# openzklib/openzl

Hardware: AMD Instinct MI355X
Metric: MSM points/sec (BLS12-381 G1) (higher is better)
Workload: dtype u32; 1 GPU; bls12_381_g1_msm_2^24_per_gpu; points_per_gpu=16777216, curve=BLS12-381 G1, scalars=uniform < r (255 bit), window_bits=20, windows=13, precomputed_table=none (the fixed-key table mode is reported separately as msm_fixed_key), parallelism=single

## Files before the change

openzl_amd/backend.py:

```python
from __future__ import annotations

import collections
import ctypes as C
import os
from typing import Optional, Tuple

import numpy as np

HERE = os.path.dirname(os.path.abspath(__file__))
LIB_PATH = os.path.join(HERE, "libzl_backend.so")

ZL_BLS12_381, ZL_BN254 = 1, 2
ZL_G1, ZL_G2 = 1, 2
ZL_MONT, ZL_COSET, ZL_INVERSE, ZL_CHECK, ZL_MONT_IN, ZL_MONT_OUT = 1, 2, 4, 8, 16, 32
ZL_PARTIAL_WORDS = 64
CURVES = {"bls12_381": ZL_BLS12_381, "bn254": ZL_BN254}
FQ_LIMBS = {ZL_BLS12_381: 6, ZL_BN254: 4}

u64p = C.POINTER(C.c_uint64)
u8p = C.POINTER(C.c_uint8)
i32p = C.POINTER(C.c_int32)

ABI_SYMBOLS = [
    "zl_ctx_create", "zl_ctx_destroy", "zl_ctx_fork", "zl_ctx_set_stream", "zl_ctx_sync", "zl_ctx_set_msm_window", "zl_ctx_last_hip_error",
# ... 744 lines not shown
            self.L.zl_mctx_destroy(self._m)
            self._m = C.c_void_p()

    def __del__(self):
        try:
            self.close()
        except Exception:
            pass


TEST_ABI_SYMBOLS = ["zl_test_poseidon_permute_dev", "zl_test_fp28_op", "zl_test_fp28_bn_op", "zl_test_pairing_product", "zl_test_point_op", "zl_test_circuit_tweak", "zl_test_fq_mul_rate", "zl_test_fr28_op", "zl_test_fr29_op",
                    "zl_test_poseidon_permute_dev28r", "zl_test_fq_mul_clock", "zl_test_acc_clock", "zl_test_acc_clock_read", "zl_test_clock_probe_launch", "zl_test_clock_probe_read",
                    "zl_test_miller_dev", "zl_test_final_exp", "zl_test_verify_batch_host", "zl_test_ntt_plan", "zl_test_ntt_fit_beside", "zl_test_fp2pair_op", "zl_test_point_form_op",
                    "zl_test_endo_split", "zl_test_endo_split_inf", "zl_test_decode_points_host", "zl_test_fq2_sqrt",
                    "zl_test_final_exp_dev", "zl_test_fq12_inverse", "zl_test_fq12_zeta", "zl_test_pairing_product_scaled",
                    "zl_test_msm_plan", "zl_test_msm_batch_form"]


def _p32(a: np.ndarray):
    assert a.dtype == np.uint32 and a.flags["C_CONTIGUOUS"]
    return a.ctypes.data_as(C.POINTER(C.c_uint32))


def groth16_keys_parse(curve: int, data: bytes, check: bool = False) -> int:
    buf = (C.c_uint8 * max(1, len(data))).from_buffer_copy(data if data else b"\0")
    return int(load_library().zl_groth16_keys_parse(curve, buf, len(data), ZL_CHECK if check else 0))


def hook_ntt_plan(log_n: int) -> list[int]:
    P = C.c_uint(0)
    sizes = (C.c_uint * 4)()
    rc = load_library().zl_test_ntt_plan(log_n, C.byref(P), sizes)
    if rc != 0:
        raise BackendError(rc, "zl_test_ntt_plan")
    assert all(sizes[k] == 0 for k in range(P.value, 4))
    return [int(sizes[k]) for k in range(P.value)]


def hook_ntt_fit_beside(be: "Backend", on: bool) -> bool:
    old = be.L.zl_test_ntt_fit_beside(be._ctx, int(on))
    if old < 0:
        raise BackendError(old, "zl_test_ntt_fit_beside")
    return bool(old)


def hook_endo_split(be: "Backend", curve: int, group: int, scalars: np.ndarray, inf: Optional[np.ndarray] = None):
    s = np.ascontiguousarray(scalars, dtype=np.uint64)
    n = s.shape[0]
    assert s.shape == (n, 4)
    out = np.zeros(4 * n * 8 + 1, dtype=np.uint32)
    k, bits = C.c_int(0), C.c_int(0)
    tail = [C.c_size_t, C.POINTER(C.c_uint32), C.POINTER(C.c_int), C.POINTER(C.c_int)]
    be.L.zl_test_endo_split.argtypes = [C.c_void_p, C.c_int, C.c_int, u64p] + tail
    be.L.zl_test_endo_split_inf.argtypes = [C.c_void_p, C.c_int, C.c_int, u64p, u8p] + tail
    if inf is None:
        rc = be.L.zl_test_endo_split(be._ctx, curve, group, _p64(s), n, _p32(out), C.byref(k), C.byref(bits))
    else:
        f = np.ascontiguousarray(inf, dtype=np.uint8)
# ... 741 lines not shown
```

openzl_amd/csrc/zl_capi.hip:

```cpp
#include <stdio.h>
#include <stdlib.h>
#include <string.h>
#include <algorithm>
#include <new>
#include <thread>
#include <vector>
#include "zl_ctx.h"
#include "zl_pool.h"
#include "zl_msm_multi_plan.h"

zl_pool& zl_pool_get() {
    static zl_pool pool(std::min(7u, std::max(1u, std::thread::hardware_concurrency()) - 1u));
    return pool;
}

int zl_ctx_aux_init(zl_ctx* ctx) {
    for (zl_ctx** ax : {&ctx->aux, &ctx->aux2}) {
        if (*ax) continue;
        zl_ctx* a = new (std::nothrow) zl_ctx();
        if (!a) return ZL_ENOMEM;
        a->device = ctx->device;
        a->cu_count = ctx->cu_count;
        int prio_lo = 0, prio_hi = 0;
        (void)hipDeviceGetStreamPriorityRange(&prio_lo, &prio_hi);
// ... 60 lines not shown
    ctx->stream = ctx->own_stream;
    const int rc_s = zl_ctx_streams_init(ctx);
    if (rc_s) { zl_ctx_destroy(ctx); return rc_s; }
    *out = ctx;
    return ZL_OK;
}

int zl_ctx_fork(zl_ctx* parent, zl_ctx** out) {
    if (!parent || !out) return ZL_EINVAL;
    *out = nullptr;
    if (parent->parent) return ZL_EINVAL;
    zl_ctx* c = nullptr;
    const int rc = zl_ctx_create(&c, parent->device);
    if (rc) return rc;
    c->msm_c = parent->msm_c;
    {
        std::unique_lock<std::shared_mutex> lk(parent->maps_mu);
        c->parent = parent;
        c->next_handle = ((uint64_t)(++parent->fork_seq) << 48) | 1;
        parent->fork_list.push_back(c);
        parent->forks.fetch_add(1);
    }
    *out = c;
    return ZL_OK;
}

int zl_ctx_drop_lanes(zl_ctx* ctx) {
    if (!ctx) return ZL_EINVAL;
    if (ctx->pipeline_busy.load()) return ZL_EINVAL;
    zl_ctx* l = ctx->stream_lane_ctx;
// ... 326 lines not shown
```

openzl_amd/csrc/zl_ctx.h:

```cpp
#pragma once
#include <hip/hip_runtime.h>
#include <stdint.h>
#include <stdlib.h>
#include <algorithm>
#include <atomic>
#include <functional>
#include <initializer_list>
#include <map>
#include <memory>
#include <mutex>
#include <shared_mutex>
#include <vector>
#include "../../include/zl_backend_ext.h"
#include "zl_curve.h"
#include "zl_pool.h"

#define ZL_HIP(ctx, call)                                   \
    do {                                                    \
        hipError_t e_ = (call);                             \
        if (e_ != hipSuccess) {                             \
            (ctx)->last_hip = (int)e_;                      \
            return e_ == hipErrorOutOfMemory ? ZL_ENOMEM : ZL_EHIP; \
        }                                                   \
    } while (0)
// ... 148 lines not shown
    size_t nnz[3] = {0, 0, 0};
    int curve = 0;
};
struct zl_ctx {
    zl_ctx* parent = nullptr;
    std::atomic<int> forks{0};
    mutable std::shared_mutex maps_mu;
    std::vector<zl_ctx*> fork_list;
    int fork_seq = 0;
    int device = 0;
    int cu_count = 0;
    hipStream_t stream = nullptr;
    hipStream_t own_stream = nullptr;
    int last_hip = 0;
    int msm_c = 0;
    int timing_on = 0;
    zl_timing timing{};
    hipEvent_t ev[4] = {nullptr, nullptr, nullptr, nullptr};
    std::map<uint64_t, zl_bases> bases;
    std::map<uint64_t, zl_r1cs_dev> r1cs;
    uint64_t next_handle = 1;
    zl_scratch scratch[ZL_SLOT_COUNT];
    std::map<uint64_t, zl_twiddles> twiddles;
    size_t ntt_last_bytes = 0;
    std::vector<hipEvent_t> ev_pool[2];
    std::atomic<int> pipeline_busy{0};
    uint64_t ntt_clock = 0;
    hipStream_t stream_sort = nullptr;
    hipStream_t stream_lane[4] = {nullptr, nullptr, nullptr, nullptr};
    hipStream_t stream_tail[3] = {nullptr, nullptr, nullptr};
// ... 125 lines not shown
```

openzl_amd/csrc/zl_msm_job.h:

```cpp
#pragma once
#include <chrono>
#include <stdlib.h>
#include <string.h>
#include <stdio.h>
#include <algorithm>
#include <vector>
#include "zl_ctx.h"
#include "zl_pool.h"
#include "zl_msm_sort.h"
#include "zl_msm_endo.h"
#include "zl_msm_accumulate.h"
#include "zl_msm_reduce.h"

#ifndef ZL_GLS_HOLE_LO_LOG
#define ZL_GLS_HOLE_LO_LOG 11
#define ZL_GLS_HOLE_HI_LOG 17
#define ZL_GLS_END_LOG 19
#endif
static_assert(ZL_GLS_HOLE_LO_LOG >= 0 && ZL_GLS_HOLE_LO_LOG <= ZL_GLS_HOLE_HI_LOG && ZL_GLS_HOLE_HI_LOG <= ZL_GLS_END_LOG && ZL_GLS_END_LOG <= 32, "split below 2^END outside [2^LO, 2^HI)");

static int zl_pick_window(size_t n, int sc_bits, bool wide16 = false ) {
    const double per_bucket = (double)zl_tune("ZL_TUNE_BUCKET_COST_X10", sc_bits > 200 ? 45 : 52) / 10.0;
    double best = 1e300;
    int best_c = 2;
// ... 9 lines not shown

static int zl_pick_window_half(size_t n_points) {
    if (n_points < 2) return 0;
    int lg = 63 - __builtin_clzll((unsigned long long)n_points);
    if ((double)n_points >= 1.4142 * (double)((size_t)1 << lg)) lg++;
    static const signed char best[9] = {9, 0, 11, 12, 0, 0, 0, 16, 0};
    return lg >= 11 && lg <= 19 ? best[lg - 11] : 0;
}
static int zl_pick_window_quarter(size_t n_points) {
    if (n_points < 2) return 0;
    int lg = 63 - __builtin_clzll((unsigned long long)n_points);
    if ((double)n_points >= 1.4142 * (double)((size_t)1 << lg)) lg++;
    static const signed char best[9] = {9, 0, 11, 12, 13, 13, 13, 13, 14};
    return lg >= 10 && lg <= 18 ? best[lg - 10] : 0;
}

static int zl_pick_window_precomp(size_t n, int sc_bits) {
    if (n < (size_t)700000) return 16;
    if (n < ((size_t)1 << 21)) return 20;
    double best = 1e300;
    int best_c = 16;
    for (int c = 20; c <= 23; c++) {
        int W = (sc_bits + 1 + c - 1) / c;
        double cost = (double)n * W + 6.0 * (double)(1u << (c - 1));
        if (cost < best) { best = cost; best_c = c; }
    }
    return best_c;
}

struct MsmSortLayout {
// ... 1 lines not shown
    uint32_t nslices = 0, per_slice = 0;
    size_t hi8 = 0, part_lo = 0, part_idx = 0, pcounts = 0, idx2 = 0, counts2 = 0;
    uint32_t P = 0, pscan_blocks = 0, fsl = 0, P2 = 0, p2scan_blocks = 0;
    size_t slice_counts = 0;
    size_t vs = 0;
};
template <class G>
struct MsmJob {
    using F = typename G::F;
    using X = XYZZ<F>;
    bool pre = false;
    int c = 0, W = 0;
    int spread_t = -1;
    bool wide = false;
    bool glv = false;
    bool phi_cached = false;
    bool phi_owner = false;
    int sc_bits = 0, endo_k = 1;
    zl_slot phi_slot = ZL_SLOT_PHI_ONE_KEY;
    MsmSortLayout lay;
    unsigned char *d_sort_a = nullptr, *d_sort_b = nullptr;
    size_t n_real = 0;
    uint32_t* d_vs = nullptr;
    const Affine<F>* d_phi = nullptr;
    uint32_t H = 0, SETS = 0, NB = 0, ZL_CHUNK = 0, nchunks = 0, scan_blocks = 0, max_big = 0, max_giant = 0, Gn = 0, big_span = ZL_BIG_SPAN;
    uint32_t red_g0 = 0, red_lg0 = 0, red_blocks = 0, red_levels = 0;
    uint32_t roots_per_set = 0;
    uint64_t maxE = 0;
    size_t n = 0, first = 0;
    const zl_bases* bsp = nullptr;
// ... 16 lines not shown
    int plan(zl_ctx* ctx, const zl_bases& bs, size_t first_, const void* d_scalars, size_t n_, zl_slot phi_slot_) {
        static const bool no_glv = getenv("ZL_NO_GLV") != nullptr;
        bool try_glv = false;
        static const size_t glv_max = (size_t)1 << zl_tune("ZL_TUNE_GLV_MAX_LOG", 19);
        if constexpr (G::GLV) try_glv = bs.precomp_c == 0 && !no_glv && n_ >= 1 && n_ <= glv_max && (uint64_t)n_ * G::ENDO_K < (1ull << 31);
        if constexpr (G::GLV && G::ENDO_K == 2) {
            if constexpr (G::GLVP::LATTICE) {
                if (n_ >= ((size_t)1 << 13) && n_ < ((size_t)1 << 17)) try_glv = false;
            }
        }
        if constexpr (G::GLV && G::ENDO_K == 4) {
            if constexpr (G::GLVP::LATTICE) {
                if (((uint64_t)n_ >= (1ull << ZL_GLS_HOLE_LO_LOG) && (uint64_t)n_ < (1ull << ZL_GLS_HOLE_HI_LOG)) || (uint64_t)n_ >= (1ull << ZL_GLS_END_LOG)) try_glv = false;
            }
        }
        int rc = plan_as(ctx, bs, first_, d_scalars, n_, try_glv);
        if (!rc && glv && c <= 3) rc = plan_as(ctx, bs, first_, d_scalars, n_, false);
        if (!rc && glv && !wide && c > 16) rc = plan_as(ctx, bs, first_, d_scalars, n_, false);
        phi_slot = phi_slot_;
        phi_owner = glv;
        return rc;
    }
    int plan_as(zl_ctx* ctx, const zl_bases& bs, size_t first_, const void* d_scalars, size_t n_, bool glv_) {
        glv = glv_;
        n_real = n_;
        endo_k = glv ? (int)G::ENDO_K : 1;
        n = (size_t)endo_k * n_;
        sc_bits = !glv ? (int)G::SC_BITS : MsmJobPartBits<G>::value;
        first = first_;
        bsp = &bs;
        pre = bs.precomp_c > 0;
        c = pre ? bs.precomp_c : (ctx->msm_c > 0 ? ctx->msm_c : zl_pick_window(n, sc_bits, glv && G::ENDO_K != 2));
        if (!pre && ctx->msm_c <= 0 && glv) {
            int h = 0;
            if constexpr (G::ENDO_K == 2) {
                if (!G::GLVP::LATTICE) h = zl_pick_window_half(n_);
            } else {
                h = zl_pick_window_quarter(n_);
            }
            if (h) c = h;
        }
        if (c < 2) c = 2;
        if (c > 24) c = 24;
        W = (sc_bits + 1 + c - 1) / c;
        H = 1u << (c - 1);
        SETS = pre ? 1u : (uint32_t)W;
        const uint64_t NB64 = (uint64_t)SETS * H;
        maxE = (uint64_t)n * W;
        if (n >= (1ull << 31) || maxE >= (1ull << 32) || NB64 >= (1ull << 31)) return ZL_EINVAL;
        if (pre && (uint64_t)W * bs.n >= (1ull << 31)) return ZL_EINVAL;
        NB = (uint32_t)NB64;
        Gn = NB >> 15;
        if (pre && (c < 16 || Gn < 1 || Gn > 255)) return ZL_EINVAL;
        wide = pre || ((c > 16 || (glv && c == 16 && G::ENDO_K != 2)) && Gn >= 1 && Gn <= 255);
        ZL_CHUNK = (maxE >> 7) >= (1u << 20) ? 128u : (uint32_t)ZL_CHUNK_MAX;
        while (ZL_CHUNK > 8 && maxE / ZL_CHUNK < (1u << 18)) ZL_CHUNK >>= 1;
        uint32_t dense = glv && G::ENDO_K == 2 ? 2u : 1u;
        if constexpr (G::GLV && G::ENDO_K == 4) {
            if constexpr (G::GLVP::LATTICE) {
                static_assert(G::GLVP::PEAK_PCT <= 400, "the top window's busiest buckets are more than 4x the average: a factor of 2 no longer keeps them below 8 chunks");
                if (glv && G::GLVP::PEAK_PCT > 200) dense = 2u;
            }
        }
        while (ZL_CHUNK < (uint32_t)ZL_CHUNK_MAX && dense * (maxE / std::max<uint64_t>(1, (uint64_t)SETS * H)) > (uint64_t)4 * ZL_CHUNK) ZL_CHUNK <<= 1;
        ZL_CHUNK = (uint32_t)std::max(8, zl_tune("ZL_TUNE_CHUNK", (int)ZL_CHUNK));
        nchunks = (uint32_t)((maxE + ZL_CHUNK - 1) / ZL_CHUNK);
        {
            uint32_t g0 = NB >= (1u << 20) ? 8u : (NB >= (1u << 17) ? 4u : 2u);
            g0 = (uint32_t)std::max(2, zl_tune("ZL_TUNE_SEG", (int)g0));
            while (g0 & (g0 - 1)) g0 &= g0 - 1;
            if (g0 > H) g0 = H;
            spread_t = -1;
            if ((wide || c <= 16) && !pre) {
                const int top_bits = sc_bits + 1 - (W - 1) * c;
                if (top_bits - 1 < c - 1) {
                    spread_t = top_bits - 1;
                    if (spread_t > 0 && (1u << spread_t) < g0) g0 = 1u << spread_t;
                }
            }
            red_g0 = g0;
            red_lg0 = 31 - __builtin_clz(g0);
            red_blocks = H / g0;
            red_levels = 31 - __builtin_clz(red_blocks);
            roots_per_set = red_levels + 2;
        }
        scan_blocks = (NB + SCAN_BLOCK * SCAN_ITEMS - 1) / (SCAN_BLOCK * SCAN_ITEMS);
        big_span = nchunks <= (1u << 17) ? (uint32_t)ZL_BIG_SPAN_SMALL : (uint32_t)ZL_BIG_SPAN;
        max_big = (uint32_t)(maxE / ((uint64_t)ZL_CHUNK * big_span)) + 1;
// ... 12 lines not shown
            lay.pcounts = lay.part_idx + b_idx;
            lay.a_bytes = lay.pcounts + up256((size_t)(2 * lay.P + lay.pscan_blocks + 8) * 4) + 256;
            lay.fsl = 16;
            while (lay.fsl * Gn < 2048 && lay.fsl < 128) lay.fsl *= 2;
            lay.P2 = Gn * 128 * lay.fsl;
            lay.p2scan_blocks = (lay.P2 + SCAN_BLOCK * SCAN_ITEMS - 1) / (SCAN_BLOCK * SCAN_ITEMS);
            lay.idx2 = b_lo;
            lay.counts2 = lay.idx2 + b_idx;
            lay.b_bytes = lay.counts2 + up256((size_t)(2 * (size_t)lay.P2 + lay.p2scan_blocks + 8) * 4) + 256;
        } else if (c <= 16) {
            lay.nslices = std::max<uint32_t>(1, std::min<uint32_t>((256 + W - 1) / W, max_slices));
            lay.slice_counts = up256((size_t)n * W * 2);
            lay.a_bytes = (size_t)n * W * 2 + (size_t)lay.nslices * NB * 4 + 256;
        }
        if (lay.nslices) lay.per_slice = (uint32_t)((n + lay.nslices - 1) / lay.nslices);
        if (glv) {
            lay.vs = up256(lay.a_bytes);
            lay.a_bytes = lay.vs + up256((size_t)n * 32);
        }
        d_bases = pre ? reinterpret_cast<const Affine<F>*>(bs.d_table) : reinterpret_cast<const Affine<F>*>(bs.d_pts) + first;
        d_inf = bs.d_inf ? reinterpret_cast<const uint8_t*>(bs.d_inf) + first : nullptr;
        sc = reinterpret_cast<const uint32_t*>(d_scalars);
        hw_own.assign((size_t)SETS * roots_per_set + 2, X::inf());
        set_host_buffer(hw_own.data());
        return ZL_OK;
    }
    bool sort_is_lds() const { return !wide && c <= 16; }
    bool lds_prefix_small() const { return NB <= 14336 && lay.nslices <= 64; }
    uint32_t lds_ranges() const {
        uint32_t ranges = 1;
        while (ranges * W < 256 && (H / (ranges * 2)) >= 64) ranges *= 2;
        return (uint32_t)std::max(1, zl_tune("ZL_TUNE_RANGES", (int)ranges));
    }
    uint32_t fine_cap() const {
// ... 79 lines not shown
            }
        }
        if (glv && phi_owner) {
            if ((rc = zl_scratch_get(ctx, phi_slot, (size_t)(endo_k - 1) * n_real * sizeof(Affine<F>), &p))) return rc;
            d_phi = reinterpret_cast<const Affine<F>*>(p);
        }
        return ZL_OK;
    }
    int sort(zl_ctx* ctx, hipStream_t st) {
        if (!wide && c > 16) ZL_HIP(ctx, hipMemsetAsync(d_counts, 0, (size_t)(NB + 1) * 4, st));
        hipLaunchKernelGGL(k_msm_zero_words, dim3(1), dim3(64), 0, st, d_big_count, 8u);
        const uint32_t nblk = (uint32_t)((n + 255) / 256);
        const uint32_t* sc_eff = sc;
        const uint8_t* inf_eff = d_inf;
        uint32_t* bad_eff = d_bad_scalar;
        if (glv) {
            d_vs = reinterpret_cast<uint32_t*>(d_sort_a + lay.vs);
            if constexpr (G::GLV && G::ENDO_K == 2) {
                if constexpr (G::GLVP::LATTICE)
                    hipLaunchKernelGGL((k_glv_split_lattice<typename G::GLVP>), dim3((uint32_t)((n_real + 255) / 256)), dim3(256), 0, st, sc, (uint32_t)n_real, d_inf, d_vs, (int)G::SC_BITS, d_bad_scalar);
                else
                    hipLaunchKernelGGL((k_glv_split<typename G::GLVP>), dim3((uint32_t)((n_real + 255) / 256)), dim3(256), 0, st, sc, (uint32_t)n_real, d_inf, d_vs, (int)G::SC_BITS, d_bad_scalar);
                if (phi_owner)
                    hipLaunchKernelGGL((k_glv_phi<G>), dim3((uint32_t)((n_real + 127) / 128)), dim3(128), 0, st, d_bases, (uint32_t)n_real, const_cast<Affine<F>*>(d_phi));
            } else if constexpr (G::GLV && G::ENDO_K == 4) {
                if constexpr (G::GLVP::LATTICE)
                    hipLaunchKernelGGL((k_gls_split_lattice<typename G::GLVP>), dim3((uint32_t)((n_real + 255) / 256)), dim3(256), 0, st, sc, (uint32_t)n_real, d_inf, d_vs, (int)G::SC_BITS, d_bad_scalar);
                else
                    hipLaunchKernelGGL((k_gls_split<typename G::GLVP>), dim3((uint32_t)((n_real + 255) / 256)), dim3(256), 0, st, sc, (uint32_t)n_real, d_inf, d_vs, (int)G::SC_BITS, d_bad_scalar);
                if (phi_owner)
                    hipLaunchKernelGGL((k_gls_psi<G>), dim3((uint32_t)((n_real + 63) / 64)), dim3(64), 0, st, d_bases, (uint32_t)n_real, const_cast<Affine<F>*>(d_phi));
// ... 11 lines not shown
        ZL_HIP(ctx, hipGetLastError());
        return ZL_OK;
    }
    void sort_wide(hipStream_t st, const uint32_t* sc_eff, const uint8_t* inf_eff, uint32_t* bad_eff, int glv_i) {
        const zl_bases& bs = *bsp;
        const uint32_t nslices = lay.nslices, per_slice = lay.per_slice, P = lay.P, pscan_blocks = lay.pscan_blocks;
        uint16_t* d_lo16 = (uint16_t*)d_sort_a;
        uint8_t* d_hi8 = (uint8_t*)(d_sort_a + lay.hi8);
        uint16_t* d_part_lo = (uint16_t*)(d_sort_a + lay.part_lo);
        uint32_t* d_part_idx = (uint32_t*)(d_sort_a + lay.part_idx);
        uint32_t* d_pcounts = (uint32_t*)(d_sort_a + lay.pcounts);
        uint32_t* d_poff = d_pcounts + P;
        uint32_t* d_pblock = d_poff + P + 1;
        const uint32_t span = 256u * std::min<uint32_t>(32u, std::max<uint32_t>(1u, (uint32_t)(n >> 19)));
        (void)hipMemsetAsync(d_pcounts, 0, (size_t)P * 4, st);
        hipLaunchKernelGGL(k_msm_recode_wide, dim3((per_slice + span - 1) / span, nslices), dim3(256), zl_recode_wide_lds(Gn, (uint32_t)W, pre ? 0u : (H >> 15)), st, sc_eff, (uint32_t)n, c, W, pre ? 0u : (H >> 15), spread_t, glv_i,
                           d_lo16, d_hi8, d_ones_list, d_ones_count, inf_eff, sc_bits, bad_eff, Gn, per_slice, span, nslices, d_pcounts);
        hipLaunchKernelGGL(k_scan_block_sums, dim3(pscan_blocks), dim3(SCAN_BLOCK), 0, st, d_pcounts, P, d_pblock);
        hipLaunchKernelGGL(k_scan_top, dim3(1), dim3(1024), 0, st, d_pblock, pscan_blocks, d_poff + P, (const uint32_t*)nullptr);
        hipLaunchKernelGGL(k_scan_apply, dim3(pscan_blocks), dim3(SCAN_BLOCK), 0, st, d_pcounts, P, d_pblock, d_poff, d_pcounts);
        hipLaunchKernelGGL(k_msm_part_scatter_st, dim3(nslices, W), dim3(256), 0, st, d_lo16, d_hi8, (uint32_t)n, (uint32_t)W, Gn, per_slice, nslices, d_poff,
                           pre ? (uint32_t)bs.n : 0u, pre ? (uint32_t)first : 0u, d_part_lo, d_part_idx);
        const uint32_t gstride = (uint32_t)W * nslices;
        const uint32_t SG = Gn * 128;
        const uint32_t fsl = lay.fsl, P2 = lay.P2, p2scan_blocks = lay.p2scan_blocks;
        uint16_t* d_lo2 = (uint16_t*)d_sort_b;
        uint32_t* d_idx2 = (uint32_t*)(d_sort_b + lay.idx2);
        uint32_t* d_c2 = (uint32_t*)(d_sort_b + lay.counts2);
        uint32_t* d_off2 = d_c2 + P2;
        uint32_t* d_blk2 = d_off2 + P2 + 1;
        hipLaunchKernelGGL(k_msm_sub_hist, dim3(fsl, Gn), dim3(256), 0, st, d_part_lo, d_poff, Gn, gstride, d_poff + P, fsl, d_c2);
// ... 155 lines not shown
            const int bsel = off - (int)red_lg0;
            if (bsel >= 0 && bsel < (int)red_levels) {
                const bool skipped = spread_t >= 0 && w == (int)SETS - 1 && off >= spread_t && !pre;
                if (!skipped) zl::add_full(v, root[2 + bsel]);
            }
            if (off == 0) zl::add_full(v, root[1]);
        }
        return v;
    }
    X finish(bool parallel = true, double* values_us = nullptr) const {
        std::vector<X> V(SETS);
        const auto t0 = std::chrono::steady_clock::now();
        if (parallel && SETS >= 4) zl_pool_get().parallel_for(SETS, [&](size_t w) { V[w] = window_value((int)w); });
        else for (uint32_t w = 0; w < SETS; w++) V[w] = window_value((int)w);
        if (values_us) *values_us = (double)std::chrono::duration_cast<std::chrono::nanoseconds>(std::chrono::steady_clock::now() - t0).count() / 1e3;
        X total = V[SETS - 1];
        for (int w = (int)SETS - 2; w >= 0; w--) {
            zl::dbl_n(total, c);
            zl::add_full(total, V[w]);
        }
        zl::add_full(total, hw[(size_t)SETS * roots_per_set]);
        return total;
    }
};
```

openzl_amd/csrc/zl_msm_sort.h:

```cpp
#pragma once
#include "zl_msm_common.h"

#define ZL_PT 4096
#define ZL_BT 16384
#define SCAN_ITEMS 16
#define SCAN_BLOCK 256

__global__ void __launch_bounds__(64) k_msm_zero_words(uint32_t* __restrict__ p, uint32_t n);
template <int MODE>
__global__ void __launch_bounds__(256) k_msm_digits(const uint32_t* __restrict__ scalars, uint32_t n, int c, int W,
                                                    uint32_t* __restrict__ counters, uint32_t* __restrict__ entries,
                                                    uint32_t* __restrict__ ones_list, uint32_t* __restrict__ ones_count, const uint8_t* __restrict__ inf,
                                                    int sc_bits, uint32_t* __restrict__ bad);
__global__ void __launch_bounds__(256) k_msm_recode(const uint32_t* __restrict__ scalars, uint32_t n, int c, int W, int spread_t, int glv, uint16_t* __restrict__ digits,
                                                             uint32_t* __restrict__ ones_list, uint32_t* __restrict__ ones_count, const uint8_t* __restrict__ inf,
                                                             int sc_bits, uint32_t* __restrict__ bad);
__global__ void __launch_bounds__(1024) k_msm_hist_lds(const uint16_t* __restrict__ digits, uint32_t n, uint32_t H, uint32_t per_slice, uint32_t NB,
                                                        uint32_t* __restrict__ counts);
__global__ void __launch_bounds__(256) k_msm_slice_prefix(uint32_t* __restrict__ counts, uint32_t NB, uint32_t nslices, uint32_t* __restrict__ tot);
__global__ void __launch_bounds__(1024) k_msm_scatter_range(const uint16_t* __restrict__ digits, uint32_t n, uint32_t H, uint32_t RB,
                                                                     const uint32_t* __restrict__ offsets, uint32_t* __restrict__ entries,
                                                                     const uint32_t* __restrict__ slice_prefix, uint32_t NB, uint32_t nslices, uint32_t per_slice,
                                                                     uint32_t parts, uint32_t W);
__global__ void __launch_bounds__(256) k_msm_recode_wide(const uint32_t* __restrict__ scalars, uint32_t n, int c, int W, uint32_t gw, int spread_t, int glv,
                                                                  uint16_t* __restrict__ lo16, uint8_t* __restrict__ hi8,
                                                                  uint32_t* __restrict__ ones_list, uint32_t* __restrict__ ones_count, const uint8_t* __restrict__ inf,
                                                                  int sc_bits, uint32_t* __restrict__ bad, uint32_t G, uint32_t per_slice, uint32_t span, uint32_t nslices,
                                                                  uint32_t* __restrict__ counts);
inline size_t zl_recode_wide_lds(uint32_t G, uint32_t W, uint32_t gw) { return (size_t)(gw ? G : G * W) * 4; }
__global__ void __launch_bounds__(256) k_msm_sub_hist(const uint16_t* __restrict__ part_lo, const uint32_t* __restrict__ part_off, uint32_t G,
                                                               uint32_t stride, const uint32_t* __restrict__ total, uint32_t fslices,
                                                               uint32_t* __restrict__ counts);
__global__ void __launch_bounds__(256) k_msm_part_scatter_st(const uint16_t* __restrict__ lo16, const uint8_t* __restrict__ hi8, uint32_t n, uint32_t W,
                                                                      uint32_t G, uint32_t per_slice, uint32_t nslices, const uint32_t* __restrict__ part_off,
                                                                      uint32_t table_stride, uint32_t first, uint16_t* __restrict__ out_lo,
                                                                      uint32_t* __restrict__ out_idx);
__global__ void __launch_bounds__(256) k_msm_sub_scatter_st(const uint16_t* __restrict__ part_lo, const uint32_t* __restrict__ part_idx,
                                                                     const uint32_t* __restrict__ part_off, uint32_t G, uint32_t stride,
                                                                     const uint32_t* __restrict__ total, uint32_t fslices, const uint32_t* __restrict__ sub_off,
                                                                     uint16_t* __restrict__ out_lo, uint32_t* __restrict__ out_idx);
__global__ void __launch_bounds__(256) k_msm_fine_hist(const uint16_t* __restrict__ lo2, const uint32_t* __restrict__ sub_off, uint32_t SG,
                                                                uint32_t fslices, const uint32_t* __restrict__ total, uint32_t* __restrict__ counts);
__global__ void __launch_bounds__(1024) k_msm_fine_sort(const uint16_t* __restrict__ lo2, const uint32_t* __restrict__ idx2,
                                                                const uint32_t* __restrict__ sub_off, uint32_t SG, uint32_t fslices,
// ... 16 lines not shown
```

openzl_amd/csrc/zl_msm_sort.hip:

```cpp
#include "zl_msm_sort.h"



__device__ __forceinline__ bool zl_take_one(const uint32_t* s, uint32_t i, uint32_t* __restrict__ ones_list, uint32_t* __restrict__ ones_count) {
    const bool one = s[0] == 1u && (s[1] | s[2] | s[3] | s[4] | s[5] | s[6] | s[7]) == 0u;
    const uint64_t m = __ballot(one);
    if (m == 0) return false;
    const uint32_t lane = threadIdx.x & 63u;
    uint32_t base = 0;
    if (lane == (uint32_t)__ffsll((long long)m) - 1u) base = atomicAdd(ones_count, (uint32_t)__popcll(m));
    base = __shfl(base, __ffsll((long long)m) - 1);
    if (one) ones_list[base + __popcll(m & ((1ull << lane) - 1ull))] = i;
    return one;
}

__device__ __forceinline__ uint32_t zl_take_sign(uint32_t& top_word, int glv) {
    if (!glv) return 0u;
    const uint32_t sg = top_word >> 31;
    top_word &= 0x7FFFFFFFu;
    return sg;
}
__global__ void __launch_bounds__(64) k_msm_zero_words(uint32_t* __restrict__ p, uint32_t n) {
    if (threadIdx.x < n) p[threadIdx.x] = 0u;
}
// ... 227 lines not shown
            uint32_t b = d - 1;
            if (spread_t >= 0 && w == W - 1) b |= (i & ((1u << (c - 1 - spread_t)) - 1u)) << spread_t;
            const uint32_t g = (uint32_t)w * gw + (b >> 15);
            lo16[(size_t)w * n + i] = (uint16_t)((b & 0x7FFFu) | ((neg ^ sg) << 15));
            hi8[(size_t)w * n + i] = d == 0 ? (uint8_t)0xFF : (uint8_t)g;
            if (d != 0 && g < G) atomicAdd(&hist[gw ? g : g * (uint32_t)W + (uint32_t)w], 1u);
        }
    }
    __syncthreads();
    for (uint32_t k = threadIdx.x; k < cells; k += blockDim.x) {
        const uint32_t v = hist[k];
        const uint32_t cell = gw ? k * (uint32_t)W + k / gw : k;
        if (v) atomicAdd(&counts[(size_t)cell * nslices + slice], v);
    }
}
__device__ __forceinline__ void zl_group_range(const uint32_t* __restrict__ part_off, uint32_t g, uint32_t G, uint32_t stride, uint32_t E, uint32_t& s,
                                               uint32_t& e) {
    s = part_off[(size_t)g * stride];
    e = (g + 1 < G) ? part_off[(size_t)(g + 1) * stride] : E;
}
__global__ void __launch_bounds__(256) k_msm_sub_hist(const uint16_t* __restrict__ part_lo, const uint32_t* __restrict__ part_off, uint32_t G,
                                                               uint32_t stride, const uint32_t* __restrict__ total, uint32_t fslices,
                                                               uint32_t* __restrict__ counts) {
    ZL_SIDE_PRIO();
    __shared__ uint32_t hist[128];
    const uint32_t slice = blockIdx.x, g = blockIdx.y;
    if (threadIdx.x < 128) hist[threadIdx.x] = 0;
    __syncthreads();
    uint32_t s, e;
    zl_group_range(part_off, g, G, stride, *total, s, e);
// ... 422 lines not shown
```

openzl_amd/csrc/zl_testhooks.hip:

```cpp
#include <string.h>
#include <type_traits>
#include <vector>
#include "../../include/zl_backend_test.h"
#include "zl_ctx.h"
#include "zl_host.h"
#include "zl_field28r.h"
#include "zl_fq2pair.h"
#include "zl_msm_endo.h"
#include "zl_decode_dev.h"

using namespace openzl;

template <class FrP>
__global__ void __launch_bounds__(64) k_test_poseidon(const uint32_t* __restrict__ keys_canon, int full_rounds, int partial_rounds, uint32_t* __restrict__ state,
                                                       uint32_t* __restrict__ disagree) {
    using F = Fp<FrP>;
    F st[3], mds[3][3];
    for (int i = 0; i < 3; i++) {
        F c;
        for (int k = 0; k < FrP::N; k++) c.l[k] = state[i * FrP::N + k];
        st[i] = zl::to_mont(c);
        for (int j = 0; j < 3; j++) mds[i][j] = zl::inv(zl::from_u64<FrP>((uint64_t)(i + 3 + j)));
    }
    const int half = full_rounds / 2;
// ... 827 lines not shown
    if (!zl_point_bytes(curve, group)) return ZL_EINVAL;
    return curve == ZL_BLS12_381 ? decode_dev::points_host_bls(group, in, count, out_xy, out_inf, status) : decode_dev::points_host_bn(group, in, count, out_xy, out_inf, status);
}
int zl_test_fq2_sqrt(zl_ctx* ctx, zl_curve_t curve, const uint64_t* in, size_t n, uint64_t* out, uint8_t* ok) {
    using namespace openzl;
    if (curve == ZL_BLS12_381) return decode_dev::fq2_sqrt_bls(ctx, in, n, out, ok);
    if (curve == ZL_BN254) return decode_dev::fq2_sqrt_bn(ctx, in, n, out, ok);
    return ZL_EINVAL;
}
int zl_test_ntt_fit_beside(zl_ctx* ctx, int on) {
    if (!ctx) return ZL_EINVAL;
    const int old = ctx->ntt_fit_beside;
    ctx->ntt_fit_beside = on ? 1 : 0;
    return old;
}

}
```

Before: 463.0 million points/s.

## Add exact-cover GLV MSM plan with variable-width windows for large inputs

Adds a new MSM planning mode for BLS12-381 G1 at 2^24 points and above. Each scalar is split on device with GLV into two 128-bit halves and recoded into six signed windows of widths 21-22 bits. The buckets of each window are grouped into sets of 2^19, and the top window only gets as many sets as its bounded digit range needs. The host recombines the sets with a doubling/running-sum scheme that uses per-set weighted sums. The aim is to cut the number of windows and buckets, and so the bucket reduction and accumulation work, compared with the generic 20-bit, 13-window non-GLV path. The cost is a new recode kernel, the phi precompute on the bases, and a more complex host-side combine.

```diff
diff --git a/openzl_amd/backend.py b/openzl_amd/backend.py
--- a/openzl_amd/backend.py
+++ b/openzl_amd/backend.py
@@ -782,7 +782,7 @@
                     "zl_test_miller_dev", "zl_test_final_exp", "zl_test_verify_batch_host", "zl_test_ntt_plan", "zl_test_ntt_fit_beside", "zl_test_fp2pair_op", "zl_test_point_form_op",
                     "zl_test_endo_split", "zl_test_endo_split_inf", "zl_test_decode_points_host", "zl_test_fq2_sqrt",
                     "zl_test_final_exp_dev", "zl_test_fq12_inverse", "zl_test_fq12_zeta", "zl_test_pairing_product_scaled",
-                    "zl_test_msm_plan", "zl_test_msm_batch_form"]
+                    "zl_test_msm_plan", "zl_test_msm_batch_form", "zl_test_msm_exact_cover"]
 
 
 def _p32(a: np.ndarray):
@@ -810,6 +810,13 @@
     if old < 0:
         raise BackendError(old, "zl_test_ntt_fit_beside")
     return bool(old)
+
+
+def hook_msm_exact_cover(be: "Backend", mode: int) -> int:
+    old = C.c_int(0)
+    be.L.zl_test_msm_exact_cover.argtypes = [C.c_void_p, C.c_int, C.POINTER(C.c_int)]
+    be._check(be.L.zl_test_msm_exact_cover(be._ctx, int(mode), C.byref(old)), "zl_test_msm_exact_cover")
+    return int(old.value)
 
 
 def hook_endo_split(be: "Backend", curve: int, group: int, scalars: np.ndarray, inf: Optional[np.ndarray] = None):
diff --git a/openzl_amd/csrc/zl_capi.hip b/openzl_amd/csrc/zl_capi.hip
--- a/openzl_amd/csrc/zl_capi.hip
+++ b/openzl_amd/csrc/zl_capi.hip
@@ -98,6 +98,7 @@
     const int rc = zl_ctx_create(&c, parent->device);
     if (rc) return rc;
     c->msm_c = parent->msm_c;
+    c->msm_cover = parent->msm_cover;
     {
         std::unique_lock<std::shared_mutex> lk(parent->maps_mu);
         c->parent = parent;
diff --git a/openzl_amd/csrc/zl_ctx.h b/openzl_amd/csrc/zl_ctx.h
--- a/openzl_amd/csrc/zl_ctx.h
+++ b/openzl_amd/csrc/zl_ctx.h
@@ -186,6 +186,7 @@
     hipStream_t own_stream = nullptr;
     int last_hip = 0;
     int msm_c = 0;
+    int msm_cover = 0;
     int timing_on = 0;
     zl_timing timing{};
     hipEvent_t ev[4] = {nullptr, nullptr, nullptr, nullptr};
diff --git a/openzl_amd/csrc/zl_msm_cover_plan.h b/openzl_amd/csrc/zl_msm_cover_plan.h
--- /dev/null
+++ b/openzl_amd/csrc/zl_msm_cover_plan.h
@@ -0,0 +1,196 @@
+#pragma once
+#include <stdint.h>
+
+#if defined(__HIPCC__)
+#define ZL_CV_HD __host__ __device__ __forceinline__
+#else
+#define ZL_CV_HD inline
+#endif
+
+#define ZL_CV_MAX_WINDOWS 8
+#define ZL_CV_BITS 128
+#define ZL_CV_GROUP_LOG 15
+
+struct zl_cover_plan {
+    uint32_t windows = 0;
+    uint32_t set_log = 0;
+    uint32_t nsets = 0;
+    uint32_t top_live = 0;
+    uint32_t width[ZL_CV_MAX_WINDOWS] = {}, pos[ZL_CV_MAX_WINDOWS] = {};
+    uint32_t base[ZL_CV_MAX_WINDOWS] = {}, sets[ZL_CV_MAX_WINDOWS] = {};
+    uint32_t lambda[4] = {}, barrett[8] = {}, rmod[8] = {};
+};
+
+enum { ZL_CV_OK = 0, ZL_CV_ESHAPE = 1, ZL_CV_ESUM = 2, ZL_CV_ECARRY = 3, ZL_CV_EGROUPS = 4 };
+
+inline int zl_cover_make(zl_cover_plan& p, const uint32_t* widths, uint32_t windows, uint32_t set_log, const uint32_t lambda[4], const uint32_t barrett[8],
+                         const uint32_t rmod[8]) {
+    p = zl_cover_plan{};
+    if (windows < 1 || windows > ZL_CV_MAX_WINDOWS || set_log < ZL_CV_GROUP_LOG || set_log > 22) return ZL_CV_ESHAPE;
+    uint32_t sum = 0;
+    for (uint32_t w = 0; w < windows; w++) {
+        if (widths[w] < set_log + 1 || widths[w] > 24) return ZL_CV_ESHAPE;
+        p.width[w] = widths[w];
+        p.pos[w] = sum;
+        sum += widths[w];
+    }
+    if (sum != ZL_CV_BITS) return ZL_CV_ESUM;
+    for (int k = 0; k < 4; k++) p.lambda[k] = lambda[k];
+    for (int k = 0; k < 8; k++) { p.barrett[k] = barrett[k]; p.rmod[k] = rmod[k]; }
+    p.windows = windows;
+    p.set_log = set_log;
+    uint32_t hm[4];
+    for (int k = 0; k < 4; k++) hm[k] = (lambda[k] >> 1) | (k < 3 ? lambda[k + 1] << 31 : 0u);
+    for (int k = 0; k < 4; k++) { hm[k] += 1u; if (hm[k] != 0u) break; }
+    if (hm[3] >> 31) return ZL_CV_ECARRY;
+    const uint32_t top = windows - 1, tp = p.pos[top];
+    uint64_t v = 0;
+    for (uint32_t k = 0; k < 4; k++) {
+        if (k == (tp >> 5)) v |= hm[k];
+        if (k == (tp >> 5) + 1) v |= (uint64_t)hm[k] << 32;
+    }
+    p.top_live = (uint32_t)(v >> (tp & 31)) + 1u;
+    if (p.top_live >= (1u << (p.width[top] - 1))) return ZL_CV_ECARRY;
+    uint32_t next = 0;
+    for (uint32_t w = 0; w < windows; w++) {
+        const uint32_t full = 1u << (p.width[w] - 1 - set_log), live = (p.top_live + (1u << set_log) - 1u) >> set_log;
+        p.base[w] = next;
+        p.sets[w] = w == top ? live : full;
+        next += p.sets[w];
+    }
+    p.nsets = next;
+    if (((uint64_t)p.nsets << (set_log - ZL_CV_GROUP_LOG)) > 255u) return ZL_CV_EGROUPS;
+    return ZL_CV_OK;
+}
+
+ZL_CV_HD uint32_t zl_cover_window_of_set(const zl_cover_plan& p, uint32_t s) {
+    uint32_t w = 0;
+#pragma unroll
+    for (uint32_t k = 1; k < ZL_CV_MAX_WINDOWS; k++)
+        if (k < p.windows && s >= p.base[k]) w = k;
+    return w;
+}
+
+struct zl_cv_u128 { uint64_t lo, hi; };
+ZL_CV_HD bool zl_cv_gt(zl_cv_u128 a, zl_cv_u128 b) { return a.hi > b.hi || (a.hi == b.hi && a.lo > b.lo); }
+ZL_CV_HD bool zl_cv_ge(zl_cv_u128 a, zl_cv_u128 b) { return a.hi > b.hi || (a.hi == b.hi && a.lo >= b.lo); }
+ZL_CV_HD zl_cv_u128 zl_cv_sub(zl_cv_u128 a, zl_cv_u128 b) { return zl_cv_u128{a.lo - b.lo, a.hi - b.hi - (a.lo < b.lo ? 1u : 0u)}; }
+ZL_CV_HD zl_cv_u128 zl_cv_inc(zl_cv_u128 a) { return zl_cv_u128{a.lo + 1, a.hi + (a.lo + 1 == 0 ? 1u : 0u)}; }
+ZL_CV_HD zl_cv_u128 zl_cv_dec(zl_cv_u128 a) { return zl_cv_u128{a.lo - 1, a.hi - (a.lo == 0 ? 1u : 0u)}; }
+
+ZL_CV_HD void zl_cover_split(const zl_cover_plan& p, const uint32_t kin[8], uint32_t mag1[4], uint32_t mag2[4], uint32_t& neg1, uint32_t& neg2) {
+    uint32_t k[8];
+    {
+        uint32_t d[8], borrow = 0;
+#pragma unroll
+        for (int w = 0; w < 8; w++) {
+            const uint64_t x = (uint64_t)kin[w] - p.rmod[w] - borrow;
+            d[w] = (uint32_t)x;
+            borrow = (uint32_t)(x >> 63);
+        }
+#pragma unroll
+        for (int w = 0; w < 8; w++) k[w] = borrow ? kin[w] : d[w];
+    }
+    uint32_t pw[16];
+    {
+        uint64_t acc = 0;
+        uint32_t top = 0;
+#pragma unroll
+        for (int col = 0; col < 15; col++) {
+#pragma unroll
+            for (int a = 0; a < 8; a++) {
+                const int b = col - a;
+                if (b < 0 || b > 7) continue;
+                const uint64_t pr = (uint64_t)k[a] * p.barrett[b];
+                acc += pr;
+                top += acc < pr ? 1u : 0u;
+            }
+            pw[col] = (uint32_t)acc;
+            acc = (acc >> 32) | ((uint64_t)top << 32);
+            top = 0;
+        }
+        pw[15] = (uint32_t)acc;
+    }
+    zl_cv_u128 q{((uint64_t)(pw[11] >> 31) | ((uint64_t)pw[12] << 1) | ((uint64_t)pw[13] << 33)), ((uint64_t)(pw[13] >> 31) | ((uint64_t)pw[14] << 1) | ((uint64_t)pw[15] << 33))};
+    const uint32_t qw[4] = {(uint32_t)q.lo, (uint32_t)(q.lo >> 32), (uint32_t)q.hi, (uint32_t)(q.hi >> 32)};
+    uint32_t t[5];
+    {
+        uint64_t acc = 0;
+        uint32_t top = 0;
+#pragma unroll
+        for (int col = 0; col < 5; col++) {
+#pragma unroll
+            for (int a = 0; a < 4; a++) {
+                const int b = col - a;
+                if (b < 0 || b > 3) continue;
+                const uint64_t pr = (uint64_t)qw[a] * p.lambda[b];
+                acc += pr;
+                top += acc < pr ? 1u : 0u;
+            }
+            t[col] = (uint32_t)acc;
+            acc = (acc >> 32) | ((uint64_t)top << 32);
+            top = 0;
+        }
+    }
+    uint32_t d[5];
+    {
+        uint32_t borrow = 0;
+#pragma unroll
+        for (int w = 0; w < 5; w++) {
+            const uint64_t x = (uint64_t)k[w] - t[w] - borrow;
+            d[w] = (uint32_t)x;
+            borrow = (uint32_t)(x >> 63);
+        }
+    }
+    const zl_cv_u128 LAM{(uint64_t)p.lambda[0] | ((uint64_t)p.lambda[1] << 32), (uint64_t)p.lambda[2] | ((uint64_t)p.lambda[3] << 32)};
+    const zl_cv_u128 HALF{(LAM.lo >> 1) | (LAM.hi << 63), LAM.hi >> 1};
+    zl_cv_u128 k1{(uint64_t)d[0] | ((uint64_t)d[1] << 32), (uint64_t)d[2] | ((uint64_t)d[3] << 32)};
+    uint32_t k1top = d[4];
+#pragma unroll
+    for (int rep = 0; rep < 2; rep++) {
+        if (k1top != 0u || zl_cv_ge(k1, LAM)) {
+            const bool br = zl_cv_gt(LAM, k1);
+            k1 = zl_cv_sub(k1, LAM);
+            k1top -= br ? 1u : 0u;
+            q = zl_cv_inc(q);
+        }
+    }
+    zl_cv_u128 k2 = q;
+    neg1 = 0;
+    neg2 = 0;
+    if (zl_cv_gt(k1, HALF)) { k1 = zl_cv_sub(LAM, k1); neg1 = 1; k2 = zl_cv_inc(k2); }
+    if (zl_cv_gt(k2, HALF)) {
+        k2 = zl_cv_sub(zl_cv_inc(LAM), k2);
+        neg2 = 1;
+        if (neg1) k1 = zl_cv_inc(k1);
+        else if ((k1.lo | k1.hi) == 0) { k1.lo = 1; neg1 = 1; }
+        else k1 = zl_cv_dec(k1);
+    }
+    if ((k1.lo | k1.hi) == 0) neg1 = 0;
+    if ((k2.lo | k2.hi) == 0) neg2 = 0;
+    mag1[0] = (uint32_t)k1.lo; mag1[1] = (uint32_t)(k1.lo >> 32); mag1[2] = (uint32_t)k1.hi; mag1[3] = (uint32_t)(k1.hi >> 32);
+    mag2[0] = (uint32_t)k2.lo; mag2[1] = (uint32_t)(k2.lo >> 32); mag2[2] = (uint32_t)k2.hi; mag2[3] = (uint32_t)(k2.hi >> 32);
+}
+
+ZL_CV_HD void zl_cover_digit(const zl_cover_plan& p, const uint32_t mag[4], uint32_t sg, uint32_t w, uint32_t& carry, uint32_t& m, uint32_t& neg) {
+    const uint32_t pos = p.pos[w], width = p.width[w], word = pos >> 5, sh = pos & 31;
+    uint64_t v = 0;
+#pragma unroll
+    for (uint32_t k = 0; k < 4; k++) {
+        if (k == word) v |= mag[k];
+        if (k == word + 1) v |= (uint64_t)mag[k] << 32;
+    }
+    uint32_t d = ((uint32_t)(v >> sh) & ((1u << width) - 1u)) + carry;
+    const uint32_t Hw = 1u << (width - 1);
+    uint32_t flip = 0;
+    carry = 0;
+    if (d > Hw - sg) { d = 2u * Hw - d; flip = 1; carry = 1; }
+    m = d;
+    neg = d ? (flip ^ sg) : 0u;
+}
+ZL_CV_HD bool zl_cover_top_ok(const zl_cover_plan& p, uint32_t top_m, uint32_t carry_out) { return carry_out == 0u && top_m <= p.top_live; }
+
+ZL_CV_HD void zl_cover_place(const zl_cover_plan& p, uint32_t w, uint32_t m, uint32_t& set, uint32_t& bucket) {
+    set = p.base[w] + ((m - 1u) >> p.set_log);
+    bucket = (m - 1u) & ((1u << p.set_log) - 1u);
+}
diff --git a/openzl_amd/csrc/zl_msm_job.h b/openzl_amd/csrc/zl_msm_job.h
--- a/openzl_amd/csrc/zl_msm_job.h
+++ b/openzl_amd/csrc/zl_msm_job.h
@@ -47,6 +47,13 @@
     static const signed char best[9] = {9, 0, 11, 12, 13, 13, 13, 13, 14};
     return lg >= 10 && lg <= 18 ? best[lg - 10] : 0;
 }
+
+#ifndef ZL_COVER_MIN_LOG
+#define ZL_COVER_MIN_LOG 24
+#endif
+#define ZL_COVER_SET_LOG 19
+static const uint32_t ZL_COVER_WIDTHS[6] = {22, 21, 21, 21, 21, 22};
+static bool zl_pick_cover(size_t n_points) { return (uint64_t)n_points >= (1ull << ZL_COVER_MIN_LOG); }
 
 static int zl_pick_window_precomp(size_t n, int sc_bits) {
     if (n < (size_t)700000) return 16;
@@ -78,6 +85,8 @@
     int spread_t = -1;
     bool wide = false;
     bool glv = false;
+    bool cover = false;
+    zl_cover_plan cv;
     bool phi_cached = false;
     bool phi_owner = false;
     int sc_bits = 0, endo_k = 1;
@@ -124,6 +133,19 @@
                 if (((uint64_t)n_ >= (1ull << ZL_GLS_HOLE_LO_LOG) && (uint64_t)n_ < (1ull << ZL_GLS_HOLE_HI_LOG)) || (uint64_t)n_ >= (1ull << ZL_GLS_END_LOG)) try_glv = false;
             }
         }
+        if constexpr (G::GLV && G::ENDO_K == 2) {
+            if constexpr (!G::GLVP::LATTICE) {
+                const bool want = ctx->msm_cover > 0 || (ctx->msm_cover == 0 && zl_pick_cover(n_));
+                if (want && bs.precomp_c == 0 && !no_glv && ctx->msm_c <= 0 && n_ >= 1 && (uint64_t)n_ * 2 * ZL_CV_MAX_WINDOWS < (1ull << 32)) {
+                    int rc = plan_as(ctx, bs, first_, d_scalars, n_, true, true);
+                    if (!rc && cover) {
+                        phi_slot = phi_slot_;
+                        phi_owner = true;
+                        return rc;
+                    }
+                }
+            }
+        }
         int rc = plan_as(ctx, bs, first_, d_scalars, n_, try_glv);
         if (!rc && glv && c <= 3) rc = plan_as(ctx, bs, first_, d_scalars, n_, false);
         if (!rc && glv && !wide && c > 16) rc = plan_as(ctx, bs, first_, d_scalars, n_, false);
@@ -131,8 +153,20 @@
         phi_owner = glv;
         return rc;
     }
-    int plan_as(zl_ctx* ctx, const zl_bases& bs, size_t first_, const void* d_scalars, size_t n_, bool glv_) {
+    int plan_as(zl_ctx* ctx, const zl_bases& bs, size_t first_, const void* d_scalars, size_t n_, bool glv_, bool cover_ = false) {
         glv = glv_;
+        cover = false;
+        if constexpr (G::GLV && G::ENDO_K == 2) {
+            if constexpr (!G::GLVP::LATTICE) {
+                if (cover_ && glv_ && bs.precomp_c == 0) {
+                    using P = typename G::GLVP;
+                    uint32_t lam[4], bar[8], rm[8];
+                    for (int k = 0; k < 4; k++) lam[k] = P::lambda(k);
+                    for (int k = 0; k < 8; k++) { bar[k] = P::barrett(k); rm[k] = P::rmod(k); }
+                    cover = zl_cover_make(cv, ZL_COVER_WIDTHS, 6, ZL_COVER_SET_LOG, lam, bar, rm) == ZL_CV_OK;
+                }
+            }
+        }
         n_real = n_;
         endo_k = glv ? (int)G::ENDO_K : 1;
         n = (size_t)endo_k * n_;
@@ -153,8 +187,12 @@
         if (c < 2) c = 2;
         if (c > 24) c = 24;
         W = (sc_bits + 1 + c - 1) / c;
+        if (cover) {
+            c = (int)cv.set_log + 1;
+            W = (int)cv.windows;
+        }
         H = 1u << (c - 1);
-        SETS = pre ? 1u : (uint32_t)W;
+        SETS = pre ? 1u : (cover ? cv.nsets : (uint32_t)W);
         const uint64_t NB64 = (uint64_t)SETS * H;
         maxE = (uint64_t)n * W;
         if (n >= (1ull << 31) || maxE >= (1ull << 32) || NB64 >= (1ull << 31)) return ZL_EINVAL;
@@ -181,7 +219,7 @@
             while (g0 & (g0 - 1)) g0 &= g0 - 1;
             if (g0 > H) g0 = H;
             spread_t = -1;
-            if ((wide || c <= 16) && !pre) {
+            if ((wide || c <= 16) && !pre && !cover) {
                 const int top_bits = sc_bits + 1 - (W - 1) * c;
                 if (top_bits - 1 < c - 1) {
                     spread_t = top_bits - 1;
@@ -224,10 +262,11 @@
             lay.a_bytes = (size_t)n * W * 2 + (size_t)lay.nslices * NB * 4 + 256;
         }
         if (lay.nslices) lay.per_slice = (uint32_t)((n + lay.nslices - 1) / lay.nslices);
-        if (glv) {
+        if (glv && !cover) {
             lay.vs = up256(lay.a_bytes);
             lay.a_bytes = lay.vs + up256((size_t)n * 32);
         }
+        if (cover && (!wide || Gn != (cv.nsets << (cv.set_log - ZL_CV_GROUP_LOG)) || Gn > 255)) return ZL_EINVAL;
         d_bases = pre ? reinterpret_cast<const Affine<F>*>(bs.d_table) : reinterpret_cast<const Affine<F>*>(bs.d_pts) + first;
         d_inf = bs.d_inf ? reinterpret_cast<const uint8_t*>(bs.d_inf) + first : nullptr;
         sc = reinterpret_cast<const uint32_t*>(d_scalars);
@@ -337,7 +376,12 @@
         const uint32_t* sc_eff = sc;
         const uint8_t* inf_eff = d_inf;
         uint32_t* bad_eff = d_bad_scalar;
-        if (glv) {
+        if (cover) {
+            if constexpr (G::GLV && G::ENDO_K == 2) {
+                if (phi_owner)
+                    hipLaunchKernelGGL((k_glv_phi<G>), dim3((uint32_t)((n_real + 127) / 128)), dim3(128), 0, st, d_bases, (uint32_t)n_real, const_cast<Affine<F>*>(d_phi));
+            }
+        } else if (glv) {
             d_vs = reinterpret_cast<uint32_t*>(d_sort_a + lay.vs);
             if constexpr (G::GLV && G::ENDO_K == 2) {
                 if constexpr (G::GLVP::LATTICE)
@@ -379,7 +423,12 @@
         uint32_t* d_pblock = d_poff + P + 1;
         const uint32_t span = 256u * std::min<uint32_t>(32u, std::max<uint32_t>(1u, (uint32_t)(n >> 19)));
         (void)hipMemsetAsync(d_pcounts, 0, (size_t)P * 4, st);
-        hipLaunchKernelGGL(k_msm_recode_wide, dim3((per_slice + span - 1) / span, nslices), dim3(256), zl_recode_wide_lds(Gn, (uint32_t)W, pre ? 0u : (H >> 15)), st, sc_eff, (uint32_t)n, c, W, pre ? 0u : (H >> 15), spread_t, glv_i,
+        if (cover) {
+            const uint32_t cspan = nslices > 1 ? std::min<uint32_t>(span, per_slice / 256u * 256u) : span;
+            hipLaunchKernelGGL(k_msm_recode_cover, dim3((uint32_t)((n_real + cspan - 1) / cspan)), dim3(256), zl_recode_cover_lds(Gn), st, sc_eff, (uint32_t)n_real, cv, d_lo16, d_hi8,
+                               d_ones_list, d_ones_count, inf_eff, (int)G::SC_BITS, bad_eff, Gn, per_slice, cspan, nslices, d_pcounts);
+        } else
+        hipLaunchKernelGGL(k_msm_recode_wide,dim3((per_slice + span - 1) / span, nslices), dim3(256), zl_recode_wide_lds(Gn, (uint32_t)W, pre ? 0u : (H >> 15)), st, sc_eff, (uint32_t)n, c, W, pre ? 0u : (H >> 15), spread_t, glv_i,
                            d_lo16, d_hi8, d_ones_list, d_ones_count, inf_eff, sc_bits, bad_eff, Gn, per_slice, span, nslices, d_pcounts);
         hipLaunchKernelGGL(k_scan_block_sums, dim3(pscan_blocks), dim3(SCAN_BLOCK), 0, st, d_pcounts, P, d_pblock);
         hipLaunchKernelGGL(k_scan_top, dim3(1), dim3(1024), 0, st, d_pblock, pscan_blocks, d_poff + P, (const uint32_t*)nullptr);
@@ -565,6 +614,26 @@
         if (parallel && SETS >= 4) zl_pool_get().parallel_for(SETS, [&](size_t w) { V[w] = window_value((int)w); });
         else for (uint32_t w = 0; w < SETS; w++) V[w] = window_value((int)w);
         if (values_us) *values_us = (double)std::chrono::duration_cast<std::chrono::nanoseconds>(std::chrono::steady_clock::now() - t0).count() / 1e3;
+        if (cover) {
+            X total = X::inf();
+            for (int w = (int)cv.windows - 1; w >= 0; w--) {
+                if (w != (int)cv.windows - 1) zl::dbl_n(total, (int)cv.width[w]);
+                X run = X::inf(), extra = X::inf(), plain = X::inf();
+                for (int j = (int)cv.sets[w] - 1; j >= 0; j--) {
+                    const uint32_t s = cv.base[w] + (uint32_t)j;
+                    zl::add_full(plain, V[s]);
+                    if (j >= 1) {
+                        zl::add_full(run, hw[(size_t)s * roots_per_set]);
+                        zl::add_full(extra, run);
+                    }
+                }
+                zl::dbl_n(extra, (int)cv.set_log);
+                zl::add_full(total, plain);
+                zl::add_full(total, extra);
+            }
+            zl::add_full(total, hw[(size_t)SETS * roots_per_set]);
+            return total;
+        }
         X total = V[SETS - 1];
         for (int w = (int)SETS - 2; w >= 0; w--) {
             zl::dbl_n(total, c);
diff --git a/openzl_amd/csrc/zl_msm_sort.h b/openzl_amd/csrc/zl_msm_sort.h
--- a/openzl_amd/csrc/zl_msm_sort.h
+++ b/openzl_amd/csrc/zl_msm_sort.h
@@ -1,5 +1,6 @@
 #pragma once
 #include "zl_msm_common.h"
+#include "zl_msm_cover_plan.h"
 
 #define ZL_PT 4096
 #define ZL_BT 16384
@@ -28,6 +29,12 @@
                                                                   int sc_bits, uint32_t* __restrict__ bad, uint32_t G, uint32_t per_slice, uint32_t span, uint32_t nslices,
                                                                   uint32_t* __restrict__ counts);
 inline size_t zl_recode_wide_lds(uint32_t G, uint32_t W, uint32_t gw) { return (size_t)(gw ? G : G * W) * 4; }
+__global__ void __launch_bounds__(256) k_msm_recode_cover(const uint32_t* __restrict__ scalars, uint32_t n_real, zl_cover_plan plan,
+                                                                   uint16_t* __restrict__ lo16, uint8_t* __restrict__ hi8,
+                                                                   uint32_t* __restrict__ ones_list, uint32_t* __restrict__ ones_count, const uint8_t* __restrict__ inf,
+                                                                   int sc_bits, uint32_t* __restrict__ bad, uint32_t G, uint32_t per_slice, uint32_t span, uint32_t nslices,
+                                                                   uint32_t* __restrict__ counts);
+inline size_t zl_recode_cover_lds(uint32_t G) { return (size_t)4 * G * 4; }
 __global__ void __launch_bounds__(256) k_msm_sub_hist(const uint16_t* __restrict__ part_lo, const uint32_t* __restrict__ part_off, uint32_t G,
                                                                uint32_t stride, const uint32_t* __restrict__ total, uint32_t fslices,
                                                                uint32_t* __restrict__ counts);
diff --git a/openzl_amd/csrc/zl_msm_sort.hip b/openzl_amd/csrc/zl_msm_sort.hip
--- a/openzl_amd/csrc/zl_msm_sort.hip
+++ b/openzl_amd/csrc/zl_msm_sort.hip
@@ -265,6 +265,76 @@
         if (v) atomicAdd(&counts[(size_t)cell * nslices + slice], v);
     }
 }
+__global__ void __launch_bounds__(256) k_msm_recode_cover(const uint32_t* __restrict__ scalars, uint32_t n_real, zl_cover_plan plan,
+                                                                   uint16_t* __restrict__ lo16, uint8_t* __restrict__ hi8,
+                                                                   uint32_t* __restrict__ ones_list, uint32_t* __restrict__ ones_count, const uint8_t* __restrict__ inf,
+                                                                   int sc_bits, uint32_t* __restrict__ bad, uint32_t G, uint32_t per_slice, uint32_t span, uint32_t nslices,
+                                                                   uint32_t* __restrict__ counts) {
+    ZL_SIDE_PRIO();
+    extern __shared__ __attribute__((aligned(16))) unsigned char smem[];
+    uint32_t* hist = reinterpret_cast<uint32_t*>(smem);
+    const uint32_t n = 2u * n_real, cells = 4u * G;
+    for (uint32_t k = threadIdx.x; k < cells; k += blockDim.x) hist[k] = 0;
+    __syncthreads();
+    const uint32_t b0 = min(n_real, blockIdx.x * span), b1 = min(n_real, b0 + span);
+    const uint32_t slice0[2] = {b0 / per_slice, (b0 + n_real) / per_slice};
+    const uint32_t edge[2] = {(slice0[0] + 1u) * per_slice, (slice0[1] + 1u) * per_slice};
+    const uint32_t gshift = plan.set_log - ZL_CV_GROUP_LOG;
+    uint4 nlo = make_uint4(0, 0, 0, 0), nhi = nlo;
+    if (b0 + threadIdx.x < b1) {
+        const uint4* sp = reinterpret_cast<const uint4*>(scalars + (size_t)(b0 + threadIdx.x) * 8);
+        nlo = sp[0]; nhi = sp[1];
+    }
+    for (uint32_t base = b0; base < b1; base += blockDim.x) {
+        const uint32_t i = base + threadIdx.x;
+        const bool live = i < b1;
+        uint4 lo = nlo, hi = nhi;
+        if (i + blockDim.x < b1) {
+            const uint4* sp = reinterpret_cast<const uint4*>(scalars + (size_t)(i + blockDim.x) * 8);
+            nlo = sp[0]; nhi = sp[1];
+        }
+        if (live) zl_flag_wide_scalar(hi.w, sc_bits, bad);
+        if (!live || (inf && inf[i])) lo = hi = make_uint4(0, 0, 0, 0);
+        const uint32_t k[8] = {lo.x, lo.y, lo.z, lo.w, hi.x, hi.y, hi.z, hi.w};
+        uint32_t mag[2][4], sgn[2];
+        zl_cover_split(plan, k, mag[0], mag[1], sgn[0], sgn[1]);
+#pragma unroll
+        for (uint32_t h = 0; h < 2; h++) {
+            const uint32_t j = i + h * n_real;
+            uint32_t rec[8] = {mag[h][0], mag[h][1], mag[h][2], mag[h][3], 0u, 0u, 0u, sgn[h] << 31};
+            if (zl_take_one(rec, j, ones_list, ones_count)) rec[0] = 0;
+            if (!live) continue;
+            const uint32_t m4[4] = {rec[0], rec[1], rec[2], rec[3]};
+            uint32_t* hh = hist + (h * 2u + (j >= edge[h] ? 1u : 0u)) * G;
+            uint32_t carry = 0;
+#pragma unroll
+            for (uint32_t w = 0; w < ZL_CV_MAX_WINDOWS; w++) {
+                if (w >= plan.windows) break;
+                uint32_t m, ng;
+                zl_cover_digit(plan, m4, sgn[h], w, carry, m, ng);
+                if (w + 1 == plan.windows && !zl_cover_top_ok(plan, m, carry)) {
+                    if (bad) atomicOr(bad, 2u);
+                    m = 0;
+                }
+                uint32_t set = 0, bucket = 0;
+                if (m) zl_cover_place(plan, w, m, set, bucket);
+                const uint32_t g = (set << gshift) | (bucket >> ZL_CV_GROUP_LOG);
+                const bool put = m != 0u && g < G;
+                lo16[(size_t)w * n + j] = (uint16_t)((bucket & 0x7FFFu) | (ng << 15));
+                hi8[(size_t)w * n + j] = put ? (uint8_t)g : (uint8_t)0xFF;
+                if (put) atomicAdd(&hh[g], 1u);
+            }
+        }
+    }
+    __syncthreads();
+    for (uint32_t c = threadIdx.x; c < cells; c += blockDim.x) {
+        const uint32_t v = hist[c];
+        if (!v) continue;
+        const uint32_t h = c / (2u * G), second = (c / G) & 1u, g = c % G;
+        const uint32_t slice = (h ? slice0[1] : slice0[0]) + second, w = zl_cover_window_of_set(plan, g >> gshift);
+        if (slice < nslices) atomicAdd(&counts[((size_t)g * plan.windows + w) * nslices + slice], v);
+    }
+}
 __device__ __forceinline__ void zl_group_range(const uint32_t* __restrict__ part_off, uint32_t g, uint32_t G, uint32_t stride, uint32_t E, uint32_t& s,
                                                uint32_t& e) {
     s = part_off[(size_t)g * stride];
diff --git a/openzl_amd/csrc/zl_testhooks.hip b/openzl_amd/csrc/zl_testhooks.hip
--- a/openzl_amd/csrc/zl_testhooks.hip
+++ b/openzl_amd/csrc/zl_testhooks.hip
@@ -865,5 +865,11 @@
     ctx->ntt_fit_beside = on ? 1 : 0;
     return old;
 }
-
-}
+int zl_test_msm_exact_cover(zl_ctx* ctx, int mode, int* old_mode) {
+    if (!ctx || mode < -1 || mode > 1) return ZL_EINVAL;
+    if (old_mode) *old_mode = ctx->msm_cover;
+    ctx->msm_cover = mode;
+    return ZL_OK;
+}
+
+}
```

Result: faster. 484.6 million points/s (median of 6 runs) (+4.7%).
